# PeihaoChen/RSPNet

Hardware: AMD Instinct MI355X
Metric: clips/sec pretext step (c3d 16x112x112, B=32/GPU) (higher is better)
Workload: dtype f32

## Files before the change

rspnet_amd/csrc/conv_igemm.hip:

```cpp
#include "common.h"
#include <algorithm>
#include <atomic>
#include <type_traits>
#include "conv_stem.h"

namespace {

constexpr int BK = 32;
constexpr int LDK = BK + 4;
constexpr int MAX_TAPS = 343;

__device__ __attribute__((aligned(64))) float g_zero[16];

const float* igemm_zero_page() {
  static const float* cache[64] = {nullptr};
  int dev = 0;
  if (hipGetDevice(&dev) != hipSuccess || dev < 0 || dev >= 64) dev = 0;
  if (!cache[dev]) {
    void* z = nullptr;
    if (hipGetSymbolAddress(&z, HIP_SYMBOL(g_zero)) != hipSuccess || !z) return nullptr;
    cache[dev] = reinterpret_cast<const float*>(z);
  }
  return cache[dev];
}
// ... 454 lines not shown
    for (int kk = 0; kk < 4; ++kk)
#pragma unroll
      for (int e = 0; e < 4; ++e)
#pragma unroll
        for (int i = 0; i < TM; ++i)
#pragma unroll
          for (int j = 0; j < TN; ++j)
            acc[i][j] = __builtin_amdgcn_mfma_f32_32x32x2f32(af[kk][i][e], bf[kk][j][e], acc[i][j], 0, 0, 0);
    if (more) store_chunk(buf ^ 1);
    __builtin_amdgcn_sched_barrier(0);
    __syncthreads();
    buf = nbuf == 1 ? 0 : buf ^ 1;
  }

  const bool linear = is_partial || p.linear_out;
  long long pwA = 0, pwD = 0;
  int pw_split = 0;
  bool piecewise = false;
  if (DMA && !linear && p.dm_dense) {
    const int P = p.Gh * p.Gw;
    const int q2a = fastdiv(m0, p.dP), f0 = m0 - q2a * P;
    pw_split = __builtin_amdgcn_readfirstlane(P - f0);
    if (BM <= pw_split + P) {
      piecewise = true;
      int n, gd;
      row_decode(p, true, q2a, n, gd);
      const int ra = (n * p.oDm + gd) * P + f0;
      row_decode(p, true, min(q2a + 1, p.Nb * p.Gd - 1), n, gd);
      const int rb = (n * p.oDm + gd) * P - pw_split;
      pwA = (long long)__builtin_amdgcn_readfirstlane(ra) * p.out_ld;
      pwD = (long long)__builtin_amdgcn_readfirstlane(rb - ra) * p.out_ld;
    }
  }
  if (!linear && !piecewise) {
    if (t < BM) {
      const int r = m0 + t;
      long long addr = -1;
      if (r < p.M) {
        const int q1 = fastdiv(r, p.dGw), gw = r - q1 * p.Gw;
        const int q2 = fastdiv(q1, p.dGh), gh = q1 - q2 * p.Gh;
        int n, gd;
        row_decode(p, DMA && p.dmajor, q2, n, gd);
        addr = ((((long long)n * p.oDm + gd * p.oSd + p.oOd) * p.oHm + gh * p.oSh + p.oOh) * p.oWm + gw * p.oSw +
                p.oOw) * p.out_ld;
      }
      rowaddr[t] = addr;
    }
    __syncthreads();
  }

  float* dst = is_partial ? p.partial : p.y;
  const long long lin_ld = is_partial ? p.Cout : p.out_ld;
  const long long lin_base = is_partial ? ((long long)z * (p.M - p.tail_row0) - p.tail_row0) * p.Cout : 0ll;
  auto store_tile = [&](auto checked, auto lin) {
    constexpr bool CHK = decltype(checked)::value, LIN = decltype(lin)::value;
#pragma unroll
    for (int j = 0; j < TN; ++j) {
      const int col = n0 + wn * WN + j * 32 + l32;
      if (col < p.Cout) {
        const float bv = (p.bias && !is_partial) ? p.bias[col] : 0.f;
        if (LIN && piecewise) {
          float* laneA = dst + pwA + (long long)(wm * WM + h * 4) * p.out_ld + col;
#pragma unroll
          for (int i = 0; i < TM; ++i)
#pragma unroll
            for (int e = 0; e < 16; ++e) {
              const int rl = wm * WM + i * 32 + (e >> 2) * 8 + h * 4 + (e & 3);
              if (!CHK || m0 + rl < p.M)
                laneA[(long long)(i * 32 + (e >> 2) * 8 + (e & 3)) * p.out_ld + (rl < pw_split ? 0ll : pwD)] = acc[i][j][e] + bv;
            }
          continue;
        }
        float* lane0 = dst + lin_base + (long long)(m0 + wm * WM + h * 4) * lin_ld + col;
#pragma unroll
        for (int i = 0; i < TM; ++i)
#pragma unroll
          for (int e = 0; e < 16; ++e) {
            const int rl = wm * WM + i * 32 + (e >> 2) * 8 + h * 4 + (e & 3);
            if (LIN) {
              if (!CHK || m0 + rl < p.M) lane0[(long long)(i * 32 + (e >> 2) * 8 + (e & 3)) * lin_ld] = acc[i][j][e] + bv;
            } else {
              const long long addr = rowaddr[rl];
              if (!CHK || addr >= 0) dst[addr + col] = acc[i][j][e] + bv;
            }
          }
      }
    }
  };
  const bool whole = m0 + BM <= p.M;
  if (linear || piecewise) {
    if (whole) store_tile(std::false_type{}, std::true_type{});
    else store_tile(std::true_type{}, std::true_type{});
  } else {
    if (whole) store_tile(std::false_type{}, std::false_type{});
    else store_tile(std::true_type{}, std::false_type{});
  }

  if (p.stat && !is_partial) {
    constexpr int SB = BM / 128;
    constexpr int WPB = WAVES_M / SB;
    static_assert(SB >= 1 && WPB >= 1 && WPB * SB == WAVES_M, "stat blocks");
    float* red = As;
#pragma unroll
    for (int j = 0; j < TN; ++j) {
      float s = 0.f, ss = 0.f;
#pragma unroll
      for (int i = 0; i < TM; ++i)
#pragma unroll
        for (int e = 0; e < 16; ++e) {
          const float v = acc[i][j][e];
          s += v;
          ss = fmaf(v, v, ss);
        }
      s += __shfl_xor(s, 32);
      ss += __shfl_xor(ss, 32);
      if (h == 0) {
        const int c = wn * WN + j * 32 + l32;
        red[(wm * BN + c) * 2 + 0] = s;
        red[(wm * BN + c) * 2 + 1] = ss;
      }
    }
    __syncthreads();
    for (int idx = t; idx < SB * BN; idx += 256) {
      const int sb = idx / BN, c = idx - sb * BN;
      if (n0 + c < p.Cout && (long long)(m_tile * SB + sb) * 128 < p.M) {
        float s = 0.f, ss = 0.f;
#pragma unroll
        for (int w = 0; w < WPB; ++w) {
          s += red[((sb * WPB + w) * BN + c) * 2 + 0];
          ss += red[((sb * WPB + w) * BN + c) * 2 + 1];
        }
        float* o = p.stat + ((long long)(m_tile * SB + sb) * p.stat_ld + n0 + c) * 2;
        o[0] = s;
        o[1] = ss;
      }
    }
  }
}

template <int BM, int BN, int WAVES_M, int WAVES_N, int VEC, int MINW = 2>
__global__ __launch_bounds__(256, MINW) void igemm_kernel(const IgemmParams p) {
  igemm_body<BM, BN, WAVES_M, WAVES_N, VEC>(p, (int)blockIdx.x, (int)gridDim.x);
}
template <int BM, int BN, int WAVES_M, int WAVES_N>
__global__ __launch_bounds__(256, 2) void igemm_ks_kernel(const IgemmParams p) {
  igemm_body<BM, BN, WAVES_M, WAVES_N, 4, true>(p, (int)blockIdx.x, (int)gridDim.x);
}

struct UnitPos {
  int m0, n0, m_tile, z, kc_begin, kc_end;
  bool is_partial;
};

template <int BM, int BN, int WAVES_M, int WAVES_N, bool KS, int FOLD = 0>
__device__ __forceinline__ void igemm_persist(const IgemmParams& p, const int wg, const int nwg, const int n_units) {
  constexpr bool HALF = BN % 32 == 16;
  constexpr int BNL = HALF ? BN + 16 : BN;
  constexpr int WM = BM / WAVES_M, WN = BNL / WAVES_N;
  constexpr int TM = WM / 32, TN = (BN / WAVES_N) / 32;
  constexpr int AR = BM / 32, BR = BNL / 32;
  static_assert(WAVES_M * WAVES_N == 4 && TM >= 1 && TN >= 1, "tile");
  static_assert(!HALF || (WAVES_N == 1 && TM == 1), "half column block: waves stacked along M, one row block each");
  constexpr int LDR = BK;
  extern __shared__ __attribute__((aligned(16))) unsigned char smem_raw[];
  const int nbuf = p.nbuf;
  const int ntaps = p.nTd * p.nTh * p.nTw;
  float* As = reinterpret_cast<float*>(smem_raw);
  float* Bs = As + nbuf * BM * LDR;
  int2* taptab = reinterpret_cast<int2*>(Bs + nbuf * BNL * LDR);
  unsigned* rowaddr = reinterpret_cast<unsigned*>(taptab + ntaps + 1);
  float* red = reinterpret_cast<float*>(rowaddr + BM);
  unsigned* xch = reinterpret_cast<unsigned*>(red + WAVES_M * BNL * 2);
  unsigned char* pblk = reinterpret_cast<unsigned char*>(xch + 4);

  const int t = threadIdx.x;
  const int lane = t & 63;
  const int wave = __builtin_amdgcn_readfirstlane(t >> 6);
  const int l32 = lane & 31, h = lane >> 5;
  const int wm = wave / WAVES_N, wn = wave % WAVES_N;
  typedef __attribute__((address_space(3))) void* lptr_t;
  {
    const int* src = reinterpret_cast<const int*>(&p);
    int* dstw = reinterpret_cast<int*>(pblk);
    for (int i = t; i < (int)(sizeof(IgemmParams) / 4); i += 256) dstw[i] = src[i];
  }
  const IgemmParams& vp = *reinterpret_cast<const IgemmParams*>(pblk);
  auto fdv = [](int n, const FastDiv& f) { return fastdiv(n, f); };
  auto row_decode_v = [&](const IgemmParams& v, bool dmajor, int q2, int& n, int& gd) { row_decode(v, dmajor, q2, n, gd); };
  for (int i = t; i < ntaps && !KS; i += 256) {
    const int q = fastdiv(i, p.dTw), aw = i - q * p.nTw;
    const int ad = fastdiv(q, p.dTh), ah = q - ad * p.nTh;
    const int od = p.off0d + ad * p.offstep, oh = p.off0h + ah * p.offstep, ow = p.off0w + aw * p.offstep;
    taptab[i] = make_int2((1 << ad) | (1 << (8 + ah)) | (1 << (16 + aw)), ((od * p.Hi + oh) * p.Wi + ow) * p.in_ld);
  }
  __amdgpu_buffer_rsrc_t rsrc_x = __builtin_amdgcn_make_buffer_rsrc(const_cast<float*>(p.x), 0, (int)p.x_bytes, 0x00020000);
  __amdgpu_buffer_rsrc_t rsrc_w = __builtin_amdgcn_make_buffer_rsrc(const_cast<float*>(p.w), 0, (int)p.w_bytes, 0x00020000);
  __amdgpu_buffer_rsrc_t rsrc_y = __builtin_amdgcn_make_buffer_rsrc(p.y, 0, (int)p.y_bytes, 0x00020000);
  __amdgpu_buffer_rsrc_t rsrc_p = __builtin_amdgcn_make_buffer_rsrc(p.partial ? p.partial : p.y, 0, (int)(p.partial ? p.partial_bytes : 4u), 0x00020000);
  const int arow = t >> 3;
  const int kcol = ((t & 7) ^ ((arow >> 1) & 7)) * 4;
  const bool tms = !KS && p.tm_skip;
  const int R = p.m_tiles * p.n_tiles - p.full_tiles;

  auto unit_pos = [&](int u) {
    UnitPos q;
    int tile;
    q.z = 0;
    q.is_partial = false;
    if (u < vp.full_tiles) {
      tile = rsp_xcd_remap(u, vp.full_tiles);
    } else {
      const int uu = rsp_xcd_remap(u - vp.full_tiles, n_units - vp.full_tiles);
      q.z = fdv(uu, vp.dR);
      tile = vp.full_tiles + (uu - q.z * R);
      q.is_partial = vp.splitk > 1;
    }
    q.m_tile = fdv(tile, vp.dNtl);
    const int n_tile = tile - q.m_tile * vp.n_tiles;
    q.m0 = q.m_tile * BM;
    q.n0 = n_tile * BN;
    q.kc_begin = q.is_partial ? q.z * vp.chunks_per_split : 0;
    q.kc_end = q.is_partial ? min(vp.nchunks, q.kc_begin + vp.chunks_per_split) : vp.nchunks;
    q.m0 = __builtin_amdgcn_readfirstlane(q.m0);
    q.n0 = __builtin_amdgcn_readfirstlane(q.n0);
    q.m_tile = __builtin_amdgcn_readfirstlane(q.m_tile);
    q.z = __builtin_amdgcn_readfirstlane(q.z);
    q.kc_begin = __builtin_amdgcn_readfirstlane(q.kc_begin);
    q.kc_end = __builtin_amdgcn_readfirstlane(q.kc_end);
    q.is_partial = __builtin_amdgcn_readfirstlane((int)q.is_partial) != 0;
    return q;
  };

  unsigned abase32[AR], rbits[AR], wrowoff[BR];
  unsigned tmask = 0x00ffffffu;
  int ld_end = 0;
  int ckc = 0;
  int ukw = 0, ukh = 0, ukd = 0, uslice = 0;
  int ntap = 0, nci = 0;
  int2 ntt = make_int2(0, 0);

  auto rows_of = [&](const UnitPos& q) {
    auto S = [](int v) { return __builtin_amdgcn_readfirstlane(v); };
    auto SF = [&](const FastDiv& f) {
      FastDiv r;
      r.mul = (unsigned)S((int)f.mul);
      r.shr = (unsigned)S((int)f.shr);
      r.d = 0;
      return r;
    };
    const int M = S(vp.M), Gw = S(vp.Gw), Gh = S(vp.Gh), Gd = S(vp.Gd), Np = S(vp.Np), dmaj = S(vp.dmajor);
    const int sD = S(vp.sD), sH = S(vp.sH), sW = S(vp.sW), Di = S(vp.Di), Hi = S(vp.Hi), Wi = S(vp.Wi), in_ld = S(vp.in_ld);
    const int o0d = S(vp.off0d), o0h = S(vp.off0h), o0w = S(vp.off0w), ostep = S(vp.offstep);
    const int nTd = S(vp.nTd), nTh = S(vp.nTh), nTw = S(vp.nTw);
    const FastDiv dGw = SF(vp.dGw), dGh = SF(vp.dGh), dGd = SF(vp.dGd), dNp = SF(vp.dNp), dGdNp = SF(vp.dGdNp);
    unsigned m_or = 0;
#pragma unroll
    for (int i = 0; i < AR; ++i) {
      const int r = q.m0 + arow + 32 * i;
      unsigned m = 0, ab = 0;
      if (r < M) {
        const int q1 = fastdiv(r, dGw), gw = r - q1 * Gw;
        const int q2 = fastdiv(q1, dGh), gh = q1 - q2 * Gh;
        int n, gd;
        if (dmaj) {
          const int part = fastdiv(q2, dGdNp);
          const int rem = q2 - part * (Gd * Np);
          const int g = fastdiv(rem, dNp);
          n = part * Np + (rem - g * Np);
          gd = g + 1 == Gd ? 0 : g + 1;
        } else {
          n = fastdiv(q2, dGd);
          gd = q2 - n * Gd;
        }
        const int id = gd * sD, ih = gh * sH, iw = gw * sW;
        ab = (unsigned)(((((long long)n * Di + id) * Hi + ih) * Wi + iw) * in_ld * 4);
        auto span = [&](int base, int D, int nT) -> unsigned {
          const int c = ostep > 0 ? base : D - 1 - base;
          const int lo = min(max(0, -c), 8), hi = min(nT - 1, D - 1 - c);
          return hi >= lo ? (2u << hi) - (1u << lo) : 0u;
        };
        m = span(id + o0d, Di, nTd) | (span(ih + o0h, Hi, nTh) << 8) | (span(iw + o0w, Wi, nTw) << 16);
      }
      abase32[i] = ab;
      rbits[i] = m;
      m_or |= m;
    }
    const int Cout = S(vp.Cout), Kld = S(vp.Kld);
#pragma unroll
    for (int i = 0; i < BR; ++i) {
      const int co = q.n0 + arow + 32 * i;
      wrowoff[i] = co < Cout ? (unsigned)co * (unsigned)Kld * 4u : 0x80000000u;
    }
    if (KS || tms) {
#pragma unroll
      for (int o = 32; o >= 1; o >>= 1) m_or |= (unsigned)__shfl_xor((int)m_or, o);
      if (lane == 0) xch[wave] = m_or;
    }
  };
  auto dead_tm = [&]() {
    if (p.cpt > 0) {
      const unsigned need = (1u << ukd) | (1u << (8 + ukh)) | (1u << (16 + ukw));
      return (tmask & need) != need;
    }
    const int t0 = fastdiv(ckc * BK, p.dCin), t1 = min(fastdiv(ckc * BK + BK - 1, p.dCin), ntaps - 1);
    const unsigned sp = (2u << fastdiv(t1, p.dThw)) - (1u << fastdiv(t0, p.dThw));
    return (tmask & sp) == 0;
  };
  auto lane_advance = [&]() {
    nci += p.adv_ci;
    ntap += p.adv_tap;
    if (nci >= p.Cin) {
      nci -= p.Cin;
      ++ntap;
    }
    ntt = taptab[min(ntap, ntaps - 1)];
// ... 240 lines not shown
        const int lim_c = cok ? lim : 0;
#pragma unroll
        for (int i = 0; i < TM; ++i)
#pragma unroll
          for (int g4 = 0; g4 < 4; ++g4) {
            const int gb = i * 32 + g4 * 8;
            const unsigned so = (unsigned)gb * pitch4;
#pragma unroll
            for (int k = 0; k < 4; ++k) {
              const float v = acc[i][j][g4 * 4 + k] + bv;
              if (MODE == 2) {
                const unsigned a = rowaddr[wm * WM + gb + h * 4 + k];
                const unsigned off = (cok && a != 0xffffffffu) ? a + (unsigned)col * 4u : 0x80000000u;
                __builtin_amdgcn_raw_buffer_store_b32(__float_as_uint(v), rs, off, 0, 0);
              } else {
                unsigned off = vo[k];
                if (MODE == 1) off += so + (gb + k < pw_lim ? 0u : pwD4);
                if (gb + k >= lim_c) off = 0x80000000u;
                __builtin_amdgcn_raw_buffer_store_b32(__float_as_uint(v), rs, off, MODE == 1 ? 0u : so, 0);
              }
            }
          }
      }
      if (HALF) {
#pragma unroll
        for (int bl = 0; bl < 2; ++bl)
#pragma unroll
          for (int k = 0; k < 4; ++k) {
            const int lrow = wm * WM + bl * 16 + g16 * 4 + k;
            const float v = acch[bl][k] + bvh;
            unsigned off;
            if (MODE == 2) {
              const unsigned a = rowaddr[lrow];
              off = (cokh && a != 0xffffffffu) ? a + (unsigned)colh * 4u : 0x80000000u;
            } else {
              off = base4 + (unsigned)lrow * pitch4 + (unsigned)colh * 4u;
              if (MODE == 1) off += lrow < pw_split ? 0u : pwD4;
              if (!cokh || q.m0 + lrow >= vp.M) off = 0x80000000u;
            }
            __builtin_amdgcn_raw_buffer_store_b32(__float_as_uint(v), rs, off, 0, 0);
          }
      }
    };
    if (vp.stat && !q.is_partial) {
      constexpr int SB = BM / 128;
      constexpr int WPB = WAVES_M / SB;
      static_assert(SB >= 1 && WPB >= 1 && WPB * SB == WAVES_M, "stat blocks");
#pragma unroll
      for (int j = 0; j < TN; ++j) {
        float s = 0.f, ss = 0.f;
#pragma unroll
        for (int i = 0; i < TM; ++i)
#pragma unroll
          for (int e = 0; e < 16; ++e) {
            const float v = acc[i][j][e];
            s += v;
            ss = fmaf(v, v, ss);
          }
        s += __shfl_xor(s, 32);
        ss += __shfl_xor(ss, 32);
        if (h == 0) {
          const int c = wn * WN + j * 32 + l32;
          red[(wm * BNL + c) * 2 + 0] = s;
          red[(wm * BNL + c) * 2 + 1] = ss;
        }
      }
      if (HALF) {
        float s = 0.f, ss = 0.f;
#pragma unroll
        for (int bl = 0; bl < 2; ++bl)
#pragma unroll
          for (int e = 0; e < 4; ++e) {
            const float v = acch[bl][e];
            s += v;
            ss = fmaf(v, v, ss);
          }
        s += __shfl_xor(s, 16);
        ss += __shfl_xor(ss, 16);
        s += __shfl_xor(s, 32);
        ss += __shfl_xor(ss, 32);
        if (g16 == 0) {
          red[(wm * BNL + TN * 32 + r16) * 2 + 0] = s;
          red[(wm * BNL + TN * 32 + r16) * 2 + 1] = ss;
        }
      }
      __syncthreads();
      for (int idx = t; idx < SB * BN; idx += 256) {
        const int sb = idx / BN, c = idx - sb * BN;
        if (q.n0 + c < vp.Cout && (long long)(q.m_tile * SB + sb) * 128 < vp.M) {
          float s = 0.f, ss = 0.f;
#pragma unroll
          for (int w = 0; w < WPB; ++w) {
            s += red[((sb * WPB + w) * BNL + c) * 2 + 0];
            ss += red[((sb * WPB + w) * BNL + c) * 2 + 1];
          }
          float* o = vp.stat + ((long long)(q.m_tile * SB + sb) * vp.stat_ld + q.n0 + c) * 2;
          o[0] = s;
          o[1] = ss;
        }
      }
    }
    if (table) store_tile(std::integral_constant<int, 2>{});
    else if (piecewise) store_tile(std::integral_constant<int, 1>{});
    else store_tile(std::integral_constant<int, 0>{});
  };

  struct HalfFrag {
    floatx4 a[2][2], b[2];
  };
  auto read_frags = [&](int buf, floatx4 (&af)[4][TM], floatx4 (&bf)[4][TN], HalfFrag& hf) {
    const float* a = As + buf * BM * LDR + (wm * WM + l32) * LDR;
    const float* b = Bs + buf * BNL * LDR + (wn * WN + l32) * LDR;
    const int swz = (l32 >> 1) & 7;
#pragma unroll
    for (int kk = 0; kk < 4; ++kk) {
      const int slot = ((h * 4 + kk) ^ swz) * 4;
#pragma unroll
      for (int i = 0; i < TM; ++i) af[kk][i] = *reinterpret_cast<const floatx4*>(a + i * 32 * LDR + slot);
#pragma unroll
      for (int j = 0; j < TN; ++j) bf[kk][j] = *reinterpret_cast<const floatx4*>(b + j * 32 * LDR + slot);
    }
    if (HALF) {
      const int r16 = lane & 15, g16 = lane >> 4;
      const int swh = (r16 >> 1) & 7;
      const float* ah = As + buf * BM * LDR + (wm * WM + r16) * LDR;
      const float* bh = Bs + buf * BNL * LDR + (TN * 32 + r16) * LDR;
#pragma unroll
      for (int hh = 0; hh < 2; ++hh) {
        const int slot = ((2 * g16 + hh) ^ swh) * 4;
        hf.a[0][hh] = *reinterpret_cast<const floatx4*>(ah + slot);
        hf.a[1][hh] = *reinterpret_cast<const floatx4*>(ah + 16 * LDR + slot);
        hf.b[hh] = *reinterpret_cast<const floatx4*>(bh + slot);
      }
    }
  };
  auto mfmas = [&](const floatx4 (&af)[4][TM], const floatx4 (&bf)[4][TN], const HalfFrag& hf) {
#pragma unroll
    for (int kk = 0; kk < 4; ++kk)
#pragma unroll
      for (int e = 0; e < 4; ++e) {
#pragma unroll
        for (int i = 0; i < TM; ++i)
#pragma unroll
          for (int j = 0; j < TN; ++j)
            acc[i][j] = __builtin_amdgcn_mfma_f32_32x32x2f32(af[kk][i][e], bf[kk][j][e], acc[i][j], 0, 0, 0);
        if (HALF && (kk & 1) == 0) {
          const int hh = kk >> 1;
#pragma unroll
          for (int bl = 0; bl < 2; ++bl)
            acch[bl] = __builtin_amdgcn_mfma_f32_16x16x4f32(hf.a[bl][hh][e], hf.b[hh][e], acch[bl], 0, 0, 0);
        }
      }
  };
  zero_acc();
  int u = wg - nwg;
  UnitPos cur = unit_pos(0);
  bool cur_valid = false, have = false;
  int buf = 0;
  __syncthreads();
  for (;;) {
    while (have && ckc < ld_end) {
      floatx4 af[4][TM], bf[4][TN];
      HalfFrag hf;
      read_frags(buf, af, bf, hf);
      const int nb = nbuf == 1 ? 0 : buf ^ 1;
      if (nbuf == 1) __syncthreads();
      load_chunk(nb);
      mfmas(af, bf, hf);
      if (FOLD > 0 && ++fold_n == FOLD) fold_panel();
      __builtin_amdgcn_sched_barrier(0);
      __syncthreads();
      buf = nb;
    }
    const bool has_next = u + nwg < n_units;
    UnitPos nxt = cur;
    if (has_next) {
      nxt = unit_pos(u + nwg);
      rows_of(nxt);
      walk_pre(nxt);
    }
    bool next_have = false;
    const int nb = nbuf == 1 ? 0 : buf ^ 1;
    if (have) {
      floatx4 af[4][TM], bf[4][TN];
      HalfFrag hf;
      read_frags(buf, af, bf, hf);
      __syncthreads();
      if (has_next) {
        walk_mask();
        next_have = ckc < ld_end;
        if (next_have) load_chunk(nb);
      }
      mfmas(af, bf, hf);
      if (FOLD > 0) {
        fold_panel();
#pragma unroll
        for (int i = 0; i < TM; ++i)
#pragma unroll
          for (int j = 0; j < TN; ++j) acc[i][j] = acc2[i][j];
      }
    } else {
      __syncthreads();
      if (has_next) {
        walk_mask();
        next_have = ckc < ld_end;
        if (next_have) load_chunk(nb);
      }
    }
    __builtin_amdgcn_sched_barrier(0);
    __syncthreads();
    buf = nb;
    if (cur_valid) epilogue(cur);
    if (!has_next) break;
    u += nwg;
    cur = nxt;
    cur_valid = true;
    have = next_have;
    zero_acc();
  }
}

template <int BM, int BN, int WAVES_M, int WAVES_N, bool KS, int MINW>
__global__ __launch_bounds__(256, MINW) void igemm_persist_kernel(const IgemmParams p, const int n_units) {
  igemm_persist<BM, BN, WAVES_M, WAVES_N, KS>(p, (int)blockIdx.x, (int)gridDim.x, n_units);
}
template <int BM, int BN, int WAVES_M, int WAVES_N, bool KS, int FOLD>
__global__ __launch_bounds__(256, 2) void igemm_persist_fold_kernel(const IgemmParams p, const int n_units) {
  igemm_persist<BM, BN, WAVES_M, WAVES_N, KS, FOLD>(p, (int)blockIdx.x, (int)gridDim.x, n_units);
}

constexpr int MAX_MULTI = 8;
struct IgemmMulti {
  int n;
  int start[MAX_MULTI + 1];
  IgemmParams p[MAX_MULTI];
};
static_assert(sizeof(IgemmMulti) <= 4096, "kernel argument segment");

template <int BM, int BN, int WAVES_M, int WAVES_N, int VEC, int MINW = 2>
__global__ __launch_bounds__(256, MINW) void igemm_multi_kernel(const IgemmMulti m) {
  int c = 0;
  while (c + 1 < m.n && (int)blockIdx.x >= m.start[c + 1]) ++c;
  igemm_body<BM, BN, WAVES_M, WAVES_N, VEC>(m.p[c], (int)blockIdx.x - m.start[c], m.start[c + 1] - m.start[c]);
}


struct DirectFrag {
  floatx4 a[4];
  floatx4 b[2][4];
};

__global__ __launch_bounds__(256, 3) void igemm_direct_kernel(const IgemmParams p) {
  __shared__ long long rowaddr[128];
  __shared__ float red[4][64][2];
  const int t = threadIdx.x, lane = t & 63;
  const int wave = __builtin_amdgcn_readfirstlane(t >> 6);
  const int l32 = lane & 31, h = lane >> 5;
  const int tiles = p.m_tiles * p.n_tiles;
  const int z = (int)blockIdx.x / tiles;
  const int tile = (int)blockIdx.x - z * tiles;
  const int m_tile = tile / p.n_tiles, n_tile = tile - m_tile * p.n_tiles;
  const int m0 = m_tile * 128, n0 = n_tile * 64;
  const bool is_partial = p.splitk > 1;
  const int kc_begin = z * p.chunks_per_split;
  const int kc_end = min(p.nchunks, kc_begin + p.chunks_per_split);
  const int ntaps = p.nTd * p.nTh * p.nTw;

  const int r = m0 + wave * 32 + l32;
  const bool rv = r < p.M;
  int n = 0, gd = 0, gh = 0, gw = 0;
  {
    const int rr = rv ? r : 0;
    const int q1 = fastdiv(rr, p.dGw);
    gw = rr - q1 * p.Gw;
    const int q2 = fastdiv(q1, p.dGh);
    gh = q1 - q2 * p.Gh;
    row_decode(p, false, q2, n, gd);
  }
  const int id0 = gd * p.sD + p.off0d, ih0 = gh * p.sH + p.off0h, iw0 = gw * p.sW + p.off0w;
  const long long xn = (long long)n * p.Di;
  const float* wrow[2];
  bool cv[2];
#pragma unroll
  for (int j = 0; j < 2; ++j) {
    const int col = n0 + j * 32 + l32;
    cv[j] = col < p.Cout;
    wrow[j] = p.w + (long long)(cv[j] ? col : 0) * p.Kld + 16 * h;
  }

  auto load = [&](int kc, DirectFrag& f) {
    const int kpos = kc * BK + 16 * h;
    int tap, ci;
    if (p.kmajor) {
      const int sl = fastdiv(kc, p.dNt);
      tap = kc - sl * ntaps;
      ci = sl * BK + 16 * h;
    } else {
      tap = fastdiv(kpos, p.dCin);
      ci = kpos - tap * p.Cin;
    }
    const bool kin = kpos < p.K;
    const int q = fastdiv(tap, p.dTw), aw = tap - q * p.nTw;
    const int ad = fastdiv(q, p.dTh), ah = q - ad * p.nTh;
    const int id = id0 + ad * p.offstep, ih = ih0 + ah * p.offstep, iw = iw0 + aw * p.offstep;
    const bool ok = rv && kin && (unsigned)id < (unsigned)p.Di && (unsigned)ih < (unsigned)p.Hi && (unsigned)iw < (unsigned)p.Wi;
    const floatx4* ap = reinterpret_cast<const floatx4*>(p.x + (((xn + id) * p.Hi + ih) * p.Wi + iw) * p.in_ld + ci);
    const floatx4 zero = {0.f, 0.f, 0.f, 0.f};
#pragma unroll
    for (int i = 0; i < 4; ++i) f.a[i] = ok ? ap[i] : zero;
#pragma unroll
    for (int j = 0; j < 2; ++j) {
      const floatx4* bp = reinterpret_cast<const floatx4*>(wrow[j] + (long long)kc * BK);
#pragma unroll
      for (int i = 0; i < 4; ++i) f.b[j][i] = (cv[j] && kin) ? bp[i] : zero;
    }
  };

  floatx16 acc[2];
#pragma unroll
  for (int j = 0; j < 2; ++j)
#pragma unroll
    for (int e = 0; e < 16; ++e) acc[j][e] = 0.f;
  auto mma = [&](const DirectFrag& f) {
#pragma unroll
    for (int i = 0; i < 4; ++i)
#pragma unroll
      for (int e = 0; e < 4; ++e)
#pragma unroll
        for (int j = 0; j < 2; ++j) acc[j] = __builtin_amdgcn_mfma_f32_32x32x2f32(f.a[i][e], f.b[j][i][e], acc[j], 0, 0, 0);
  };

  DirectFrag f0, f1;
  if (kc_begin < kc_end) load(kc_begin, f0);
  for (int kc = kc_begin; kc < kc_end; kc += 2) {
    if (kc + 1 < kc_end) load(kc + 1, f1);
    mma(f0);
    if (kc + 1 < kc_end) {
      if (kc + 2 < kc_end) load(kc + 2, f0);
      mma(f1);
    }
  }

  if (!is_partial && !p.linear_out) {
    if (t < 128) {
      const int rr = m0 + t;
      long long addr = -1;
      if (rr < p.M) {
        const int q1 = fastdiv(rr, p.dGw), w_ = rr - q1 * p.Gw;
        const int q2 = fastdiv(q1, p.dGh), h_ = q1 - q2 * p.Gh;
        int n_, d_;
        row_decode(p, false, q2, n_, d_);
        addr = ((((long long)n_ * p.oDm + d_ * p.oSd + p.oOd) * p.oHm + h_ * p.oSh + p.oOh) * p.oWm + w_ * p.oSw + p.oOw) * p.out_ld;
      }
      rowaddr[t] = addr;
    }
    __syncthreads();
  }
  float* dst = is_partial ? p.partial + (long long)z * p.M * p.Cout : p.y;
  const long long ld = is_partial ? p.Cout : p.out_ld;
#pragma unroll
  for (int j = 0; j < 2; ++j) {
    const int col = n0 + j * 32 + l32;
    if (col < p.Cout) {
      const float bv = (p.bias && !is_partial) ? p.bias[col] : 0.f;
#pragma unroll
      for (int e = 0; e < 16; ++e) {
        const int rl = wave * 32 + (e >> 2) * 8 + h * 4 + (e & 3);
        if (m0 + rl < p.M) {
          const long long addr = (is_partial || p.linear_out) ? (long long)(m0 + rl) * ld : rowaddr[rl];
          dst[addr + col] = acc[j][e] + bv;
        }
      }
    }
  }
  if (p.stat && !is_partial) {
#pragma unroll
    for (int j = 0; j < 2; ++j) {
// ... 221 lines not shown
  __shared__ float tile[4096 + 64];
  __shared__ int tsrc_of[MAX_TAPS];
  float* __restrict__ row = out + (long long)o * j.Kld;
  for (int tap = threadIdx.x; tap < j.ntaps; tap += 256) {
    const int aw = tap % j.nTw, q = tap / j.nTw;
    const int ah = q % j.nTh, ad = q / j.nTh;
    tsrc_of[tap] = ((j.k0d + ad * j.kstepd) * j.kH + (j.k0h + ah * j.ksteph)) * j.kW + (j.k0w + aw * j.kstepw);
  }
  const int T = j.kT * j.kH * j.kW;
  const bool kmaj = k_slice_major(j.C, j.ntaps);
  const int CH = T >= 4096 ? 1 : (4096 / T > 128 ? 128 : 4096 / T);
  const bool o_in = o < (j.transpose ? j.Cin_src : j.Cout_src);
  const int c_in = j.transpose ? j.Cout_src : j.Cin_src;
  const long long fbase = j.transpose ? (long long)o * T : (long long)o * j.Cin_src * T;
  const long long fstride = j.transpose ? (long long)j.Cin_src * T : (long long)T;
  for (int c0 = 0; c0 < j.C; c0 += CH) {
    const int nc = min(CH, j.C - c0);
    __syncthreads();
    const int nel = nc * T;
    if (!j.transpose) {
      const float* __restrict__ src = w + fbase + (long long)c0 * T;
      const int lim = o_in ? min(nel, max(0, c_in - c0) * T) : 0;
      for (int e = threadIdx.x; e < nel; e += 256) tile[e] = e < lim ? src[e] : 0.f;
    } else {
      int cl = (int)threadIdx.x / T, t = (int)threadIdx.x - cl * T;
      const int dcl = 256 / T, dt = 256 - dcl * T;
      for (int e = threadIdx.x; e < nel; e += 256) {
        const int c = c0 + cl;
        tile[e] = (o_in && c < c_in) ? w[fbase + c * fstride + t] : 0.f;
        cl += dcl;
        t += dt;
        if (t >= T) {
          t -= T;
          ++cl;
        }
      }
    }
    __syncthreads();
    {
      int tap = (int)threadIdx.x / nc, cl = (int)threadIdx.x - tap * nc;
      const int dtap = 256 / nc, dcl = 256 - dtap * nc;
      for (int e = threadIdx.x; e < j.ntaps * nc; e += 256) {
        row[k_index(kmaj, tap, c0 + cl, j.C, j.ntaps)] = tile[cl * T + tsrc_of[tap]];
        tap += dtap;
        cl += dcl;
        if (cl >= nc) {
          cl -= nc;
          ++tap;
        }
      }
    }
  }
  for (int k = j.ntaps * j.C + threadIdx.x; k < j.Kld; k += 256) row[k] = 0.f;
}

template <int BM, int BN, int WAVES_M, int WAVES_N>
int launch_ks_cfg(const IgemmParams& p, hipStream_t s) {
  const size_t lds = (size_t)p.nbuf * (BM + BN) * BK * sizeof(float) + (size_t)(p.nTd * p.nTh * p.nTw + 1) * sizeof(int4) + BM * sizeof(long long);
  static bool attr_set = false;
  if (!attr_set) {
    const size_t lds_max = (size_t)2 * (BM + BN) * BK * sizeof(float) + (MAX_TAPS + 1) * sizeof(int4) + BM * sizeof(long long);
    (void)hipFuncSetAttribute(reinterpret_cast<const void*>(&igemm_ks_kernel<BM, BN, WAVES_M, WAVES_N>),
                              hipFuncAttributeMaxDynamicSharedMemorySize, (int)lds_max);
    attr_set = true;
  }
  dim3 grid(p.full_tiles + (p.m_tiles * p.n_tiles - p.full_tiles) * p.splitk);
  rsp_note_kernel("igemm_ks_kernel<%d, %d, %d, %d>", BM, BN, WAVES_M, WAVES_N);
  hipLaunchKernelGGL((igemm_ks_kernel<BM, BN, WAVES_M, WAVES_N>), grid, dim3(256), lds, s, p);
  return rsp_check_launch("igemm_ks_kernel");
}

template <int BM, int BN, int WAVES_M, int WAVES_N, int VEC, int MINW = 2>
int launch_cfg(const IgemmParams& p, hipStream_t s) {
  const size_t nb = VEC == 4 ? (size_t)p.nbuf : 2;
  const size_t lds = nb * (BM + BN) * (VEC == 4 ? BK : LDK) * sizeof(float) +
                     (size_t)(p.nTd * p.nTh * p.nTw + 1) * sizeof(int4) + BM * sizeof(long long);
  static bool attr_set = false;
  if (!attr_set) {
    const size_t lds_max = (size_t)2 * (BM + BN) * (VEC == 4 ? BK : LDK) * sizeof(float) + (MAX_TAPS + 1) * sizeof(int4) +
                           BM * sizeof(long long);
    (void)hipFuncSetAttribute(reinterpret_cast<const void*>(&igemm_kernel<BM, BN, WAVES_M, WAVES_N, VEC, MINW>),
                        hipFuncAttributeMaxDynamicSharedMemorySize, (int)lds_max);
    attr_set = true;
  }
  dim3 grid(p.full_tiles + (p.m_tiles * p.n_tiles - p.full_tiles) * p.splitk);
  rsp_note_kernel("igemm_kernel<%d, %d, %d, %d, %d, %d>", BM, BN, WAVES_M, WAVES_N, VEC, MINW);
  hipLaunchKernelGGL((igemm_kernel<BM, BN, WAVES_M, WAVES_N, VEC, MINW>), grid, dim3(256), lds, s, p);
  return rsp_check_launch("igemm_kernel");
}

inline int tile_bn(int Cout) {
  if (Cout > 128 && Cout <= 160) return 160;
  if (Cout > 64 && Cout <= 96) return 96;
  return Cout > 64 ? 128 : (Cout > 32 ? 64 : 32);
}

std::atomic<int> g_narrow_max_tiles{-1};
static int narrow_max_tiles() {
  const int set = g_narrow_max_tiles.load(std::memory_order_relaxed);
  if (set >= 0) return set;
  static const int v = getenv("RSP_NARROW_MAX_TILES") ? atoi(getenv("RSP_NARROW_MAX_TILES")) : 512;
  return v;
}
std::atomic<int> g_narrow32_max_units{-1};
static int narrow32_max_units() {
  const int set = g_narrow32_max_units.load(std::memory_order_relaxed);
  if (set >= 0) return set;
  static const int v = getenv("RSP_NARROW32_MAX_UNITS") ? atoi(getenv("RSP_NARROW32_MAX_UNITS")) : 256;
  return v;
}
inline int narrow_bn(long long M, int Cout, int nchunks) {
  const long long mt = rsp_cdiv(M, 128);
  if (Cout > 32 && nchunks >= 8 && mt * rsp_cdiv(Cout, 64) <= narrow32_max_units()) return 32;
  const bool cols = Cout > 160 || (Cout > 96 && Cout <= 128);
  return (cols && mt * rsp_cdiv(Cout, 128) < narrow_max_tiles()) ? 64 : 0;
}
inline int tile_bn_of(const IgemmParams& p) { return p.bn_narrow ? p.bn_narrow : tile_bn(p.Cout); }

std::atomic<int> g_tall_min_tiles{-1};
static int tall_min_tiles() {
  const int set = g_tall_min_tiles.load(std::memory_order_relaxed);
  if (set >= 0) return set;
  static const int v = getenv("RSP_TALL_MIN_TILES") ? atoi(getenv("RSP_TALL_MIN_TILES")) : 0;
  return v;
}
inline bool tall_tiles(long long M, int bn, bool vec4) {
  const int lim = tall_min_tiles();
  return vec4 && bn == 64 && lim > 0 && M / 256 >= lim;
}

template <int BM, int BN, int WAVES_M, int WAVES_N, int VEC, int MINW = 2>
int launch_multi_cfg(const IgemmMulti& m, int max_taps, hipStream_t s) {
  const size_t lds = (size_t)2 * (BM + BN) * BK * sizeof(float) + (size_t)(max_taps + 1) * sizeof(int4) + BM * sizeof(long long);
  static bool attr_set = false;
  if (!attr_set) {
    const size_t lds_max = (size_t)2 * (BM + BN) * BK * sizeof(float) + (MAX_TAPS + 1) * sizeof(int4) + BM * sizeof(long long);
    (void)hipFuncSetAttribute(reinterpret_cast<const void*>(&igemm_multi_kernel<BM, BN, WAVES_M, WAVES_N, VEC, MINW>),
                              hipFuncAttributeMaxDynamicSharedMemorySize, (int)lds_max);
    attr_set = true;
  }
  rsp_note_kernel("igemm_multi_kernel<%d, %d, %d, %d, %d, %d>", BM, BN, WAVES_M, WAVES_N, VEC, MINW);
  hipLaunchKernelGGL((igemm_multi_kernel<BM, BN, WAVES_M, WAVES_N, VEC, MINW>), dim3(m.start[m.n]), dim3(256), lds, s, m);
  return rsp_check_launch("igemm_multi_kernel");
}


constexpr int persist_minw(int bn, int bm = 128) { return bm > 128 ? 3 : (bn > 128 ? 2 : (bn > 64 ? 3 : 4)); }

static bool persist_enabled() {
  static const bool off = getenv("RSP_NO_PERSIST") != nullptr;
  return !off;
}

template <int BM, int BN, int WAVES_M, int WAVES_N, bool KS>
int launch_persist_cfg(const IgemmParams& p, hipStream_t s) {
  constexpr int MINW = persist_minw(BN, BM);
  const int ntaps = p.nTd * p.nTh * p.nTw;
  constexpr int BNL = (BN + 31) / 32 * 32;
  auto lds_of = [&](int nbuf, int taps) {
    return (size_t)nbuf * (BM + BNL) * BK * sizeof(float) + (size_t)(taps + 2) / 2 * sizeof(int4) + BM * sizeof(unsigned) +
           (size_t)WAVES_M * BNL * 2 * sizeof(float) + 4 * sizeof(unsigned) + sizeof(IgemmParams);
  };
  const size_t lds = lds_of(p.nbuf, ntaps);
  static bool attr_set = false;
  if (!attr_set) {
    (void)hipFuncSetAttribute(reinterpret_cast<const void*>(&igemm_persist_kernel<BM, BN, WAVES_M, WAVES_N, KS, MINW>),
                              hipFuncAttributeMaxDynamicSharedMemorySize, (int)lds_of(2, MAX_TAPS));
    attr_set = true;
  }
  const int n_units = p.full_tiles + (p.m_tiles * p.n_tiles - p.full_tiles) * p.splitk;
  int wpc = (int)(160 * 1024 / lds);
  wpc = wpc > MINW ? MINW : (wpc < 1 ? 1 : wpc);
  int G = 256 * wpc;
  if (n_units <= G) G = n_units;
  rsp_note_kernel("igemm_persist_kernel<%d, %d, %d, %d, %s, %d>", BM, BN, WAVES_M, WAVES_N, KS ? "true" : "false", MINW);
  hipLaunchKernelGGL((igemm_persist_kernel<BM, BN, WAVES_M, WAVES_N, KS, MINW>), dim3(G), dim3(256), lds, s, p, n_units);
  return rsp_check_launch("igemm_persist_kernel");
}

constexpr int FOLD_CHUNKS = 16;
std::atomic<int> g_two_level_min_chunks{-1};
static int two_level_min_chunks() {
  const int set = g_two_level_min_chunks.load(std::memory_order_relaxed);
  if (set >= 0) return set;
  static const int v = getenv("RSP_TWO_LEVEL_MIN_CHUNKS") ? atoi(getenv("RSP_TWO_LEVEL_MIN_CHUNKS")) : 0;
  return v;
}

template <int BM, int BN, int WAVES_M, int WAVES_N, bool KS, int FOLD>
int launch_persist_fold_cfg(const IgemmParams& p, hipStream_t s) {
  const int ntaps = p.nTd * p.nTh * p.nTw;
  auto lds_of = [&](int nbuf, int taps) {
    return (size_t)nbuf * (BM + BN) * BK * sizeof(float) + (size_t)(taps + 2) / 2 * sizeof(int4) + BM * sizeof(unsigned) +
           (size_t)WAVES_M * BN * 2 * sizeof(float) + 4 * sizeof(unsigned) + sizeof(IgemmParams);
  };
  const size_t lds = lds_of(p.nbuf, ntaps);
  static bool attr_set = false;
  if (!attr_set) {
    (void)hipFuncSetAttribute(reinterpret_cast<const void*>(&igemm_persist_fold_kernel<BM, BN, WAVES_M, WAVES_N, KS, FOLD>),
                              hipFuncAttributeMaxDynamicSharedMemorySize, (int)lds_of(2, MAX_TAPS));
    attr_set = true;
  }
  const int n_units = p.full_tiles + (p.m_tiles * p.n_tiles - p.full_tiles) * p.splitk;
  int wpc = (int)(160 * 1024 / lds);
  wpc = wpc > 2 ? 2 : (wpc < 1 ? 1 : wpc);
  int G = 256 * wpc;
  if (n_units <= G) G = n_units;
  rsp_note_kernel("igemm_persist_fold_kernel<%d, %d, %d, %d, %s, %d>", BM, BN, WAVES_M, WAVES_N, KS ? "true" : "false", FOLD);
  hipLaunchKernelGGL((igemm_persist_fold_kernel<BM, BN, WAVES_M, WAVES_N, KS, FOLD>), dim3(G), dim3(256), lds, s, p, n_units);
  return rsp_check_launch("igemm_persist_fold_kernel");
}

static bool half_block_cols(int cols) {
  static const bool off = getenv("RSP_NO_HALF_BLOCK") != nullptr;
  return !off && cols > 128 && cols <= 144;
}
static bool half_block(const IgemmParams& p) { return half_block_cols(p.Cout); }

int launch_persist(IgemmParams& p, hipStream_t s) {
  const int bn = tile_bn_of(p);
  const int bm = p.bm > 128 ? 256 : 128;
  p.m_tiles = rsp_cdiv(p.M, bm);
  p.n_tiles = rsp_cdiv(p.Cout, bn);
  const int R = p.m_tiles * p.n_tiles - p.full_tiles;
  p.dR = fastdiv_make(R > 0 ? R : 1);
  p.dNtl = fastdiv_make(p.n_tiles);
  if (bm == 256) {
    if (bn != 64) {
      rsp_set_error("launch_persist: the 256-row tile is 64 columns wide");
      return RSP_EINVAL;
    }
    return p.kmajor ? launch_persist_cfg<256, 64, 4, 1, true>(p, s) : launch_persist_cfg<256, 64, 4, 1, false>(p, s);
  }
  if (p.kmajor) {
    if (bn == 128 && two_level_min_chunks() > 0 && p.nchunks >= two_level_min_chunks())
      return launch_persist_fold_cfg<128, 128, 2, 2, true, FOLD_CHUNKS>(p, s);
    switch (bn) {
      case 160: return half_block(p) ? launch_persist_cfg<128, 144, 4, 1, true>(p, s) : launch_persist_cfg<128, 160, 4, 1, true>(p, s);
      case 128: return launch_persist_cfg<128, 128, 2, 2, true>(p, s);
      case 96: return launch_persist_cfg<128, 96, 4, 1, true>(p, s);
      case 64: return launch_persist_cfg<128, 64, 2, 2, true>(p, s);
      default: return launch_persist_cfg<128, 32, 4, 1, true>(p, s);
    }
  }
  switch (bn) {
    case 160: return half_block(p) ? launch_persist_cfg<128, 144, 4, 1, false>(p, s) : launch_persist_cfg<128, 160, 4, 1, false>(p, s);
    case 128: return launch_persist_cfg<128, 128, 2, 2, false>(p, s);
    case 96: return launch_persist_cfg<128, 96, 4, 1, false>(p, s);
    case 64: return launch_persist_cfg<128, 64, 2, 2, false>(p, s);
    default: return launch_persist_cfg<128, 32, 4, 1, false>(p, s);
  }
}

static unsigned out_extent_bytes(const IgemmParams& p) {
  const unsigned long long pos = (unsigned long long)p.Nb * p.oDm * p.oHm * p.oWm;
  const unsigned long long b = ((pos - 1) * (unsigned long long)p.out_ld + (unsigned long long)p.Cout) * 4ull;
  return b < 0x7ffffff0ull ? (unsigned)b : 0u;
}

inline void fill_fastdiv_linear(IgemmParams& p) {
  const bool dense = p.oSd == 1 && p.oSh == 1 && p.oSw == 1 && p.oOd == 0 && p.oOh == 0 && p.oOw == 0 && p.oDm == p.Gd &&
                     p.oHm == p.Gh && p.oWm == p.Gw;
  p.linear_out = dense && !p.dmajor;
  p.dm_dense = dense && p.dmajor;
  p.dP = fastdiv_make(p.Gh * p.Gw);
}

inline void fill_fastdiv(IgemmParams& p) {
  p.dGw = fastdiv_make(p.Gw); p.dGh = fastdiv_make(p.Gh); p.dGd = fastdiv_make(p.Gd);
  p.dCin = fastdiv_make(p.Cin); p.dTw = fastdiv_make(p.nTw); p.dTh = fastdiv_make(p.nTh);
  p.adv_tap = BK / p.Cin;
  p.adv_ci = BK % p.Cin;
  p.kmajor = k_slice_major(p.Cin, p.nTd * p.nTh * p.nTw) ? 1 : 0;
  static const bool no_skip = getenv("RSP_NO_PAD_SKIP") != nullptr;
  static const bool no_dmajor = getenv("RSP_NO_DMAJOR") != nullptr;
  p.skip_pad = no_skip ? 0 : 1;
  p.Np = (p.Nb % 8 == 0 && (long long)(p.Nb / 8) * p.Gh * p.Gw >= 4 * 128) ? p.Nb / 8 : (p.Nb > 0 ? p.Nb : 1);
  p.dNp = fastdiv_make(p.Np);
  p.dGdNp = fastdiv_make(p.Gd * p.Np);
  const int dlo = p.offstep > 0 ? p.off0d : p.off0d - (p.nTd - 1);
  const int dhi = (p.Gd - 1) * p.sD + (p.offstep > 0 ? p.off0d + p.nTd - 1 : p.off0d);
  const int ntaps = p.nTd * p.nTh * p.nTw;
  p.cpt = p.Cin % BK == 0 ? p.Cin / BK : 0;
  static const bool no_tm = getenv("RSP_NO_TM_SKIP") != nullptr;
  p.dThw = fastdiv_make(p.nTh * p.nTw);
  p.tm_skip = (p.skip_pad && !no_tm && !p.kmajor && p.nTd > 1 && (dlo < 0 || dhi >= p.Di)) ? 1 : 0;
  const long long tiles_est = ((long long)p.M + 127) / 128 * ((p.Cout + 127) / 128);
  const bool wants_dmajor = (long long)p.Gh * p.Gw < 4 * 128 || tiles_est < 8 * 768;
  p.dmajor = (p.skip_pad && !no_dmajor && (p.kmajor || p.tm_skip) && wants_dmajor && p.nTd > 1 && p.Gd > 1 && p.Nb > 1 &&
              (dlo < 0 || dhi >= p.Di)) ? 1 : 0;
  (void)ntaps;
  p.dNt = fastdiv_make(p.nTd * p.nTh * p.nTw);
  fill_fastdiv_linear(p);
}

int launch_igemm(IgemmParams& p, bool vec4, hipStream_t s) {
  int bn = tile_bn_of(p);
  if (!vec4 && (bn == 160 || bn == 96)) bn = 128;
  p.m_tiles = rsp_cdiv(p.M, 128);
  p.n_tiles = rsp_cdiv(p.Cout, bn);
  if (vec4 && p.kmajor) {
    switch (bn) {
      case 160: return launch_ks_cfg<128, 160, 4, 1>(p, s);
      case 128: return launch_ks_cfg<128, 128, 2, 2>(p, s);
      case 96: return launch_ks_cfg<128, 96, 4, 1>(p, s);
      case 64: return launch_ks_cfg<128, 64, 2, 2>(p, s);
      default: return launch_ks_cfg<128, 32, 4, 1>(p, s);
    }
  }
  if (bn == 160) return launch_cfg<128, 160, 4, 1, 4>(p, s);
  if (bn == 96) return launch_cfg<128, 96, 4, 1, 4>(p, s);
  if (bn == 128) return vec4 ? launch_cfg<128, 128, 2, 2, 4>(p, s) : launch_cfg<128, 128, 2, 2, 1>(p, s);
  if (bn == 64) return vec4 ? launch_cfg<128, 64, 2, 2, 4>(p, s) : launch_cfg<128, 64, 2, 2, 1>(p, s);
  return vec4 ? launch_cfg<128, 32, 4, 1, 4>(p, s) : launch_cfg<128, 32, 4, 1, 1>(p, s);
}

struct SplitPlan {
  int full_tiles;
  int splitk;
  int cps;
};

bool single_buffer(int m_tiles, int n_tiles, int bn, bool vec4) {
  return vec4 && (bn == 128 || bn == 96) && (long long)m_tiles * n_tiles >= 768;
}

SplitPlan plan_split(int m_tiles, int n_tiles, int bn, bool vec4, int nchunks, int Cout, int bm = 128) {
  const int tiles = m_tiles * n_tiles;
// ... 924 lines not shown
```

Measured before the change: 351.9.

## Software-pipeline persistent igemm K loop to overlap LDS fragment reads with MFMAs

Adds a PIPE variant of the persistent implicit-GEMM kernel for single-buffer configs (BM=128, WAVES_M=2, BN 128 or 64, split-K). The K loop is split into four quarter-steps. The LDS reads for the next chunk's first quarter are issued while the previous chunk's last quarter of MFMAs is still running, and the global-to-LDS load is placed between MFMA quarters. The aim is to hide LDS read latency and barrier stalls that the serial read-then-compute loop exposes. The cost is more live fragment registers and a more rigid schedule. An RSP_NO_KPIPE environment variable turns the variant off.

```diff
diff --git a/rspnet_amd/csrc/conv_igemm.hip b/rspnet_amd/csrc/conv_igemm.hip
--- a/rspnet_amd/csrc/conv_igemm.hip
+++ b/rspnet_amd/csrc/conv_igemm.hip
@@ -630,7 +630,7 @@
   bool is_partial;
 };
 
-template <int BM, int BN, int WAVES_M, int WAVES_N, bool KS, int FOLD = 0>
+template <int BM, int BN, int WAVES_M, int WAVES_N, bool KS, int FOLD = 0, bool PIPE = false>
 __device__ __forceinline__ void igemm_persist(const IgemmParams& p, const int wg, const int nwg, const int n_units) {
   constexpr bool HALF = BN % 32 == 16;
   constexpr int BNL = HALF ? BN + 16 : BN;
@@ -639,6 +639,7 @@
   constexpr int AR = BM / 32, BR = BNL / 32;
   static_assert(WAVES_M * WAVES_N == 4 && TM >= 1 && TN >= 1, "tile");
   static_assert(!HALF || (WAVES_N == 1 && TM == 1), "half column block: waves stacked along M, one row block each");
+  static_assert(!PIPE || (!HALF && FOLD == 0), "pipelined K loop: whole 32-wide column blocks, one summation level");
   constexpr int LDR = BK;
   extern __shared__ __attribute__((aligned(16))) unsigned char smem_raw[];
   const int nbuf = p.nbuf;
@@ -1185,14 +1186,67 @@
         }
       }
   };
+  auto read_q = [&](int kk, floatx4 (&af)[4][TM], floatx4 (&bf)[4][TN]) {
+    const float* a = As + (wm * WM + l32) * LDR;
+    const float* b = Bs + (wn * WN + l32) * LDR;
+    const int slot = ((h * 4 + kk) ^ ((l32 >> 1) & 7)) * 4;
+#pragma unroll
+    for (int i = 0; i < TM; ++i) af[kk][i] = *reinterpret_cast<const floatx4*>(a + i * 32 * LDR + slot);
+#pragma unroll
+    for (int j = 0; j < TN; ++j) bf[kk][j] = *reinterpret_cast<const floatx4*>(b + j * 32 * LDR + slot);
+  };
+  auto mfma_q = [&](int kk, const floatx4 (&af)[4][TM], const floatx4 (&bf)[4][TN]) {
+#pragma unroll
+    for (int e = 0; e < 4; ++e)
+#pragma unroll
+      for (int i = 0; i < TM; ++i)
+#pragma unroll
+        for (int j = 0; j < TN; ++j)
+          acc[i][j] = __builtin_amdgcn_mfma_f32_32x32x2f32(af[kk][i][e], bf[kk][j][e], acc[i][j], 0, 0, 0);
+  };
+  auto read_under_q3 = [&](floatx4 (&af)[4][TM], floatx4 (&bf)[4][TN]) {
+    read_q(0, af, bf);
+    __builtin_amdgcn_sched_barrier(0);
+    mfma_q(3, af, bf);
+    __builtin_amdgcn_sched_barrier(0);
+    read_q(1, af, bf);
+    read_q(2, af, bf);
+    read_q(3, af, bf);
+    __builtin_amdgcn_sched_barrier(0);
+  };
   zero_acc();
   int u = wg - nwg;
   UnitPos cur = unit_pos(0);
   bool cur_valid = false, have = false;
   int buf = 0;
+  floatx4 paf[4][TM], pbf[4][TN];
   __syncthreads();
   for (;;) {
-    while (have && ckc < ld_end) {
+    if (PIPE && have && ckc < ld_end) {
+      HalfFrag hf;
+      read_frags(0, paf, pbf, hf);
+      __syncthreads();
+      load_chunk(0);
+      mfma_q(0, paf, pbf);
+      mfma_q(1, paf, pbf);
+      mfma_q(2, paf, pbf);
+      __builtin_amdgcn_sched_barrier(0);
+      __syncthreads();
+      while (ckc < ld_end) {
+        read_under_q3(paf, pbf);
+        mfma_q(0, paf, pbf);
+        __builtin_amdgcn_sched_barrier(0);
+        __syncthreads();
+        load_chunk(0);
+        mfma_q(1, paf, pbf);
+        mfma_q(2, paf, pbf);
+        __builtin_amdgcn_sched_barrier(0);
+        __syncthreads();
+      }
+      mfma_q(3, paf, pbf);
+      __builtin_amdgcn_sched_barrier(0);
+    }
+    while (!PIPE && have && ckc < ld_end) {
       floatx4 af[4][TM], bf[4][TN];
       HalfFrag hf;
       read_frags(buf, af, bf, hf);
@@ -1253,9 +1307,9 @@
   }
 }
 
-template <int BM, int BN, int WAVES_M, int WAVES_N, bool KS, int MINW>
+template <int BM, int BN, int WAVES_M, int WAVES_N, bool KS, int MINW, bool PIPE = false>
 __global__ __launch_bounds__(256, MINW) void igemm_persist_kernel(const IgemmParams p, const int n_units) {
-  igemm_persist<BM, BN, WAVES_M, WAVES_N, KS>(p, (int)blockIdx.x, (int)gridDim.x, n_units);
+  igemm_persist<BM, BN, WAVES_M, WAVES_N, KS, 0, PIPE>(p, (int)blockIdx.x, (int)gridDim.x, n_units);
 }
 template <int BM, int BN, int WAVES_M, int WAVES_N, bool KS, int FOLD>
 __global__ __launch_bounds__(256, 2) void igemm_persist_fold_kernel(const IgemmParams p, const int n_units) {
@@ -1783,6 +1837,11 @@
   return !off;
 }
 
+static bool kpipe_enabled() {
+  static const bool off = getenv("RSP_NO_KPIPE") != nullptr;
+  return !off;
+}
+
 template <int BM, int BN, int WAVES_M, int WAVES_N, bool KS>
 int launch_persist_cfg(const IgemmParams& p, hipStream_t s) {
   constexpr int MINW = persist_minw(BN, BM);
@@ -1805,6 +1864,12 @@
   int G = 256 * wpc;
   if (n_units <= G) G = n_units;
   rsp_note_kernel("igemm_persist_kernel<%d, %d, %d, %d, %s, %d>", BM, BN, WAVES_M, WAVES_N, KS ? "true" : "false", MINW);
+  if constexpr (KS && BM == 128 && WAVES_M == 2 && (BN == 128 || BN == 64)) {
+    if (p.nbuf == 1 && kpipe_enabled()) {
+      hipLaunchKernelGGL((igemm_persist_kernel<BM, BN, WAVES_M, WAVES_N, KS, MINW, true>), dim3(G), dim3(256), lds, s, p, n_units);
+      return rsp_check_launch("igemm_persist_kernel");
+    }
+  }
   hipLaunchKernelGGL((igemm_persist_kernel<BM, BN, WAVES_M, WAVES_N, KS, MINW>), dim3(G), dim3(256), lds, s, p, n_units);
   return rsp_check_launch("igemm_persist_kernel");
 }
```

Result: faster. 356.7, median of 6 (+1.4%).
